# AHzZ123/orb_slam2_with_comment

Hardware: AMD Instinct MI355X
Metric: frames/sec (Track+LocalMap) on 1241×376 stereo; kpts+desc/sec at 1/2/4/8 GPUs (higher is better)
Workload: dtype u8; 1 GPU; Track+LocalMap per stereo frame: ORBextractor(L,R) [2000 feat, 1.2, 8 lv, FAST 20/7] + ComputeStereoMatches + TrackWithMotionModel [SearchByProjection(CF,LF,th=7), PoseOptimization] + TrackLocalMap [SearchLocalPoints(th=1, ~1971 MPs), PoseOptimization] + LocalMapping::Run every 4th frame on the concurrent LocalMapping thread [ProcessNewKeyFrame: KeyFrame::ComputeBoW (a queued keyframe's issued bes; frames_resident=8, parallelism=one stereo stream per GPU x1

## Files before the change

orb_slam2_with_comment_amd/csrc/lba.hip:

```cpp
#include <algorithm>
#include <cfloat>
#include <chrono>
#include <cstdio>
#include <cstdlib>
#include <cmath>
#include <cstring>
#include <new>
#include <thread>
#include <vector>

#include "extractor.h"
#include "se3_device.h"
#include "wave_ops.h"

#if defined(__HIP_DEVICE_COMPILE__) && !defined(__gfx950__)
#error "lba.hip's fence-free fan-ins are validated on gfx950 only"
#endif

#pragma clang fp contract(fast)

namespace orbmi {

constexpr int kBaMaxPoses = 30;
constexpr int kBaMaxN = 6 * kBaMaxPoses;
// ... 172 lines not shown
    edge_robust_math(fl, ed, edge_chi2_math(ed, err), &r0, &r1);
    *w = (fl & 2) ? info : r1 * info;
    const double s = (fl & 2) ? 1.0 : r1;
    for (int k = 0; k < 3; k++) om[k] = -(info * err[k]) * s;
}

__device__ inline void edge_error_at(const BaDev& a, int i, const double* T, const double* Xp, double* err) {
    const orbmi_ba_edge e = a.edges[i];
    edge_err_math(e, ba_cam(a.kfs[e.kf]), T + 8 * e.kf, Xp, err);
}

__device__ inline void edge_error(const BaDev& a, int i, const double* T, const double* X, double* err) {
    edge_error_at(a, i, T, X + 4 * a.edges[i].point, err);
}

__device__ inline double edge_chi2(const BaDev& a, int i) { return edge_chi2_math(a.edges[i], a.err + 3 * i); }

__device__ inline void edge_robust(const BaDev& a, int i, double c, double* rho0, double* rho1) {
    edge_robust_math(a.eflag[i], a.edges[i], c, rho0, rho1);
}

template <int NT>
__device__ inline double block_sum(double v, double* red) {
    for (int o = 32; o > 0; o >>= 1) v += __shfl_xor(v, o, 64);
    if ((threadIdx.x & 63) == 0) red[threadIdx.x >> 6] = v;
    __syncthreads();
    double t = 0;
    for (int w = 0; w < NT / 64; w++) t += red[w];
    __syncthreads();
    return t;
}

template <int NT>
__device__ inline void block_sum2_t0(double& x, double& y, double* red ) {
    for (int o = 32; o > 0; o >>= 1) {
        x += __shfl_xor(x, o, 64);
        y += __shfl_xor(y, o, 64);
    }
    if ((threadIdx.x & 63) == 0) {
        red[threadIdx.x >> 6] = x;
        red[NT / 64 + (threadIdx.x >> 6)] = y;
    }
    __syncthreads();
    if (threadIdx.x == 0) {
        x = 0;
        y = 0;
        for (int w = 0; w < NT / 64; w++) x += red[w];
        for (int w = 0; w < NT / 64; w++) y += red[NT / 64 + w];
    }
}

template <int NT>
__device__ inline double block_max(double v, double* red) {
    for (int o = 32; o > 0; o >>= 1) v = fmax(v, __shfl_xor(v, o, 64));
    if ((threadIdx.x & 63) == 0) red[threadIdx.x >> 6] = v;
    __syncthreads();
    double t = 0;
    for (int w = 0; w < NT / 64; w++) t = fmax(t, red[w]);
    __syncthreads();
    return t;
}

__device__ inline int packed(int r, int c, int N) { return r * N - r * (r - 1) / 2 + (c - r); }

__host__ __device__ inline int mfma_tile_pos(int T, int R, int C) {
    const int i = R >> 4, j = C >> 4, rr = R & 15;
    return (i * (T + 1) - i * (i - 1) / 2 + (j - i)) * 256 + (rr >> 2) * 64 + 16 * (rr & 3) + (C & 15);
}


__device__ inline bool point_active(const BaDev& a, int p) {
    for (int i = a.pt_start[p]; i < a.pt_start[p + 1]; i++)
        if (a.eflag[i] & 4) return true;
    return false;
}

__device__ inline bool ba_check_stop(const BaDev& a, BaCtl& c) {
    const int idx = c.checks++;
    const bool s = (a.stop && *a.stop) || (a.stop_at >= 0 && idx >= a.stop_at);
    if (s && c.stop_seen < 0) c.stop_seen = idx;
    return s;
}

__global__ __launch_bounds__(kBaBlock) void k_ba_setup(BaDev a, double* __restrict__ T, double* __restrict__ X,
                                                       unsigned char* __restrict__ out_erase) {
    const int i = blockIdx.x * blockDim.x + threadIdx.x;
    if (i == 0) {
        BaCtl c = {};
        c.checks = 1;
        c.stop_seen = -1;
        *a.ctl = c;
        for (int k = 0; k < 8; k++) a.istat[k] = 0;
    }
    if (i < a.nkf) {
        const float* t = a.kfs[i].tcw;
        double R[3][3];
        for (int r = 0; r < 3; r++)
            for (int c = 0; c < 3; c++) R[r][c] = t[4 * r + c];
        Q q = q_from_matrix(R);
        q_normalize(q);
        double* Ti = T + 8 * i;
        Ti[0] = q.x; Ti[1] = q.y; Ti[2] = q.z; Ti[3] = q.w; Ti[4] = t[3]; Ti[5] = t[7]; Ti[6] = t[11]; Ti[7] = 0;
        a.kf_act[i] = 0;
    }
    if (i < a.nf) a.arrive_kf[i] = 0;
    if (i < a.npt) {
        for (int r = 0; r < 3; r++) X[4 * i + r] = a.pts[i].pos[r];
        X[4 * i + 3] = 0;
    }
    if (i < a.nedge) {
        a.eflag[i] = 0;
        out_erase[i] = 0;
        a.err[3 * i] = a.err[3 * i + 1] = a.err[3 * i + 2] = 0;
    }
}

__global__ __launch_bounds__(kBaBlock) void k_ba_levels(BaDev a) {
    if (!(a.ctl->phases_done >= 1 && a.ctl->do_more)) return;
    const int i = blockIdx.x * blockDim.x + threadIdx.x;
    const double* T = a.Tb[a.ctl->cur];
    const double* X = a.Xb[a.ctl->cur];
    if (i >= a.nedge) return;
    const orbmi_ba_edge e = a.edges[i];
    if (a.pts[e.point].bad) return;
    double p[3];
    se3_map(T + 8 * e.kf, X + 4 * e.point, p);
    const double th = edge_stereo(e) ? 7.815 : 5.991;
    unsigned char f = a.eflag[i] & 3;
    if (edge_chi2(a, i) > th || !(p[2] > 0.0)) f |= 1;
    f |= 2;
    a.eflag[i] = f;
}

__device__ inline void activate_ctl_body(const BaDev& a, int max_it, int gen);
__global__ __launch_bounds__(kBaBlock) void k_ba_activate_edges(BaDev a, int max_it, int gen) {
    if (gen > 1 && !(a.ctl->phases_done >= gen - 1 && a.ctl->do_more)) return;
    __shared__ double red[kBaBlock / 64];
    const int i = blockIdx.x * blockDim.x + threadIdx.x;
    int first = 0;
    if (i < a.nedge) {
        unsigned char f = a.eflag[i] & 3;
        if (!(f & 1)) {
            f |= 4;
            const orbmi_ba_edge e = a.edges[i];
            a.kf_act[e.kf] = gen;
            first = 1;
            for (int j = a.pt_start[e.point]; j < i; j++)
                if (!(a.eflag[j] & 1)) { first = 0; break; }
        }
        a.eflag[i] = f;
    }
    const double n = block_sum<kBaBlock>((double)first, red);
    __shared__ bool last;
    if (threadIdx.x == 0) {
        a.part_lin[blockIdx.x] = n;
        __threadfence();
        last = atomicAdd(&a.ctl->arrive_e, 1u) == gridDim.x - 1;
    }
    __syncthreads();
    if (!last) return;
    __threadfence();
    if (threadIdx.x < 64) activate_ctl_body(a, max_it, gen);
    if (threadIdx.x == 0) a.ctl->arrive_e = 0;
}

__device__ inline void activate_ctl_body(const BaDev& a, int max_it, int gen) {
    const int lane = threadIdx.x;
    double c = 0;
    for (int b = lane; b < a.nb_e; b += 64) c += a.part_lin[b];
    const int nl = (int)wave_sum(c);
    int n = 0;
    for (int o0 = 0; o0 < a.nkf; o0 += 64) {
        const int oi = o0 + lane;
        int k = -1;
        bool take = false;
        if (oi < a.nkf) {
            k = a.kf_order[oi];
            take = !a.kfs[k].fixed && a.kf_act[k] == gen;
        }
        const unsigned long long m = __ballot(take);
        const int idx = n + __popcll(m & ((1ull << lane) - 1));
        if (k >= 0) {
            a.pose_idx[k] = take && idx < kBaMaxPoses ? idx : -1;
            if (take && idx < kBaMaxPoses) a.pose_kf[idx] = k;
        }
        n += __popcll(m);
    }
    if (lane == 0) {
        a.istat[0] = n;
        a.istat[1] = nl;
        a.istat[2] = n > kBaMaxPoses;
        BaCtl& c2 = *a.ctl;
        c2.np = min(n, kBaMaxPoses);
        c2.nl = nl;
        c2.unsupported |= n > kBaMaxPoses;
// ... 1310 lines not shown
        for (int e = pe0 + j; e < pe1; e += kBaUpdLanes) {
            act += (a.eflag[e] & 4) ? 1.0 : 0.0;
            const int i1 = a.e_pi[e];
            if (i1 < 0) continue;
            const double* B = y.Hpl + 18 * (long long)e;
            const double* xp = a.xp + 6 * i1;
#pragma unroll
            for (int r = 0; r < 6; r++) {
                c0 += B[r * 3] * xp[r];
                c1 += B[r * 3 + 1] * xp[r];
                c2 += B[r * 3 + 2] * xp[r];
            }
        }
        c0 = sum8(c0); c1 = sum8(c1); c2 = sum8(c2); act = sum8(act);
        if (own && j == 0) {
            double xl[3] = {0, 0, 0};
            if (ok && act > 0) {
                const double cl[3] = {y.bl[3 * p] - c0, y.bl[3 * p + 1] - c1, y.bl[3 * p + 2] - c2};
                double Di[9];
                point_dinv(y.Hll, p, lam, Di);
                for (int r = 0; r < 3; r++) xl[r] = Di[r * 3] * cl[0] + Di[r * 3 + 1] * cl[1] + Di[r * 3 + 2] * cl[2];
            }
            for (int r = 0; r < 3; r++) {
                const double x = X[4 * p + r] + xl[r];
                Xt[4 * p + r] = x;
                xs[ps][r] = x;
                if (ok) sc += xl[r] * (lam * xl[r] + y.bl[3 * p + r]);
            }
        }
    }
    __syncthreads();
    const bool lds = be1 - be0 <= kBaUpdLdsEdges;
    for (int e = e_pre; e < be1; e += blockDim.x) {
        EdgeIn s;
        if (e == e_pre) s = pre;
        else edge_in(a, e, Tt, s);
        chi += edge_trial(a, t, e, s, &xs[s.e.point - p0][0], lds ? sHe + 9 * (e - be0) : nullptr);
    }
    __syncthreads();
    {
        double h[9] = {0, 0, 0, 0, 0, 0, 0, 0, 0};
        for (int e = pe0 + j; e < pe1; e += kBaUpdLanes) {
            if (!(a.eflag[e] & 4)) continue;
            const double* He = lds ? sHe + 9 * (e - be0) : t.Hle + 9 * (long long)e;
#pragma unroll
            for (int k = 0; k < 9; k++) h[k] += He[k];
        }
#pragma unroll
        for (int k = 0; k < 9; k++) h[k] = sum8(h[k]);
        if (own && j == 0) {
            double* H = t.Hll + 9 * p;
            H[0] = h[0]; H[1] = h[1]; H[2] = h[2];
            H[3] = h[1]; H[4] = h[3]; H[5] = h[4];
            H[6] = h[2]; H[7] = h[4]; H[8] = h[5];
            for (int k = 0; k < 3; k++) t.bl[3 * p + k] = h[6 + k];
        }
    }
    block_sum2_t0<kBaUpdThreads>(chi, sc, red);
    if (tid == 0) {
        __hip_atomic_store(&part_chi[blockIdx.x], chi, __ATOMIC_RELAXED, __HIP_MEMORY_SCOPE_AGENT);
        __hip_atomic_store(&part_scale[blockIdx.x], sc, __ATOMIC_RELAXED, __HIP_MEMORY_SCOPE_AGENT);
        asm volatile("s_waitcnt vmcnt(0)" ::: "memory");
        last = atomicAdd(&ctl.arrive, 1u) == gridDim.x - 1;
    }
    __syncthreads();
    if (!last) return;
    if (tid < 64) k_ba_control_body(a);
    if (tid == 0) ctl.arrive = 0;
}

__device__ inline void chi_body(const BaDev& a, int phase) {
    const double chi = wave_sum_fixed_sc1(a.part_lin, a.nb_e);
    if (threadIdx.x == 0) {
        BaCtl& c = *a.ctl;
        c.chi_out[phase] = chi;
        c.it_out[phase] = (c.np + c.nl == 0) ? -1 : c.it;
        c.phases_done = phase + 1;
        if (phase == 0) c.do_more = !ba_check_stop(a, c);
    }
}

__global__ __launch_bounds__(kBaBlock) void k_ba_finish(BaDev a, float* __restrict__ out_tcw,
                                                        float* __restrict__ out_pos,
                                                        unsigned char* __restrict__ out_erase) {
    const int i = blockIdx.x * blockDim.x + threadIdx.x;
    const double* T = a.Tb[a.ctl->cur];
    const double* X = a.Xb[a.ctl->cur];
    if (i < a.nedge) {
        const orbmi_ba_edge e = a.edges[i];
        if (!a.pts[e.point].bad) {
            double p[3];
            se3_map(T + 8 * e.kf, X + 4 * e.point, p);
            const double th = edge_stereo(e) ? 7.815 : 5.991;
            out_erase[i] = (edge_chi2(a, i) > th || !(p[2] > 0.0)) ? 1 : 0;
        }
    }
    if (i < a.nkf) {
        const double* Ti = T + 8 * i;
        double R[3][3];
        q_to_matrix(load_q(Ti), R);
        float* o = out_tcw + 16 * i;
        for (int r = 0; r < 3; r++) {
            for (int c = 0; c < 3; c++) o[4 * r + c] = (float)R[r][c];
            o[4 * r + 3] = (float)Ti[4 + r];
        }
        o[12] = 0; o[13] = 0; o[14] = 0; o[15] = 1;
    }
    if (i < a.npt)
        for (int r = 0; r < 3; r++) out_pos[3 * i + r] = (float)X[4 * i + r];
}

}

struct orbmi_ba {
    int device = 0;
    hipStream_t stream = nullptr;
    bool own_stream = true;
    hipEvent_t done = nullptr;
    uint8_t* d_buf = nullptr;
    size_t cap = 0;
    uint8_t* h_stage = nullptr;
    size_t cap_stage = 0;
    hipEvent_t up_done = nullptr;
    hipStream_t up_stream = nullptr;
    uint8_t* h_out = nullptr;
    size_t cap_out = 0;
    orbmi::BaCtl* h_ctl = nullptr;
    int* h_stop = nullptr;
    int* d_stop = nullptr;
    int stop_at = -1;
    void (*enqueued)(void*) = nullptr;
    void* enqueued_arg = nullptr;
};

namespace {

using namespace orbmi;

struct BaTrace {
    bool on = getenv("ORBMI_BA_TRACE") != nullptr;
    std::chrono::steady_clock::time_point t0 = std::chrono::steady_clock::now(), last = t0;
    char buf[512];
    int n = 0;
    void mark(const char* what) {
        if (!on) return;
        const auto t = std::chrono::steady_clock::now();
        n += snprintf(buf + n, sizeof(buf) - n > 0 ? sizeof(buf) - n : 0, " %s %.1f", what,
                      std::chrono::duration<double, std::micro>(t - last).count());
        last = t;
    }
    ~BaTrace() {
        if (on) fprintf(stderr, "[ba] total %.1f us:%s\n",
                        std::chrono::duration<double, std::micro>(std::chrono::steady_clock::now() - t0).count(), buf);
    }
};

inline bool stop_set(const volatile int* stop) { return stop && __atomic_load_n(stop, __ATOMIC_ACQUIRE) != 0; }

bool ba_block_table(int nf, std::vector<int>& blk_id) {
    const int nblk = nf * (nf + 1) / 2;
    blk_id.assign(std::max(nblk, 1), -1);
    const int R = 8;
    std::vector<int> load(R, 0), grp(std::max(nf, 1));
    for (int r = 0; r < nf; r++) {
        const int g = (int)(std::min_element(load.begin(), load.end()) - load.begin());
        grp[r] = g;
        load[g] += nf - r;
    }
    std::vector<int> next(R);
    for (int g = 0; g < R; g++) next[g] = g;
    std::vector<char> used(std::max(nblk, 1), 0);
    std::vector<int> spill;
    int l = 0;
    for (int ra = 0; ra < nf; ra++)
        for (int rb = ra; rb < nf; rb++, l++) {
            const int g = grp[ra];
            if (next[g] < nblk) { blk_id[l] = next[g]; used[next[g]] = 1; next[g] += R; }
            else spill.push_back(l);
        }
    int free_id = 0;
    for (int x : spill) {
        while (free_id < nblk && used[free_id]) free_id++;
        if (free_id >= nblk) return false;
        blk_id[x] = free_id;
        used[free_id] = 1;
    }
    std::vector<char> hit(std::max(nblk, 1), 0);
    for (int x = 0; x < nblk; x++) {
        const int id = blk_id[x];
        if (id < 0 || id >= nblk || hit[id]) return false;
        hit[id] = 1;
    }
    return true;
}

constexpr int kBaStepSlack = 1;

struct Runner {
    orbmi_ba& h;
    BaDev a;
    const volatile int* stop;

    void launch_solve() {
        static_assert((6 * kBaSolveMfmaMaxPoses + 15) / 16 <= 8, "a case per tile count below");
        switch (a.mfma_T) {
#define ORBMI_MFMA_CASE(T_) \
    case T_: hipLaunchKernelGGL(k_ba_solve_mfma<T_>, dim3(1), dim3(kBaMfmaThreads), 0, h.stream, a); break;
            ORBMI_MFMA_CASE(1) ORBMI_MFMA_CASE(2) ORBMI_MFMA_CASE(3) ORBMI_MFMA_CASE(4)
            ORBMI_MFMA_CASE(5) ORBMI_MFMA_CASE(6) ORBMI_MFMA_CASE(7) ORBMI_MFMA_CASE(8)
#undef ORBMI_MFMA_CASE
            default: hipLaunchKernelGGL(k_ba_solve, dim3(1), dim3(kBaSolveThreads), 0, h.stream, a); break;
        }
    }

    int wait() {
        ORBMI_HIP(hipEventRecord(h.done, h.stream));
        if (!stop) {
            ORBMI_HIP(hipEventSynchronize(h.done));
            return ORBMI_OK;
        }
        for (;;) {
            *(volatile int*)h.h_stop = stop_set(stop) ? 1 : 0;
            const hipError_t e = hipEventQuery(h.done);
            if (e == hipSuccess) return ORBMI_OK;
            if (e != hipErrorNotReady) return ORBMI_E_HIP;
            std::this_thread::yield();
        }
    }

    int read_ctl() {
        ORBMI_HIP(hipMemcpyAsync(h.h_ctl, a.ctl, sizeof(BaCtl), hipMemcpyDeviceToHost, h.stream));
        return wait();
    }

    void step(int gen) {
        a.run_gen = gen;
        if (a.nblk > 0)
            hipLaunchKernelGGL(k_ba_schur, dim3(a.nblk + kSchurKfSplit * a.nf + (a.mfma_T > 0)), dim3(kSchurThreads), 0,
                               h.stream, a);
        launch_solve();
        hipLaunchKernelGGL(k_ba_update_errors, dim3(a.nb_q), dim3(kBaUpdThreads), 0, h.stream, a);
    }

    void prologue(int iterations, int gen) {
        a.run_gen = gen;
        if (gen == 2) hipLaunchKernelGGL(k_ba_levels, dim3(a.nb_e), dim3(kBaBlock), 0, h.stream, a);
        hipLaunchKernelGGL(k_ba_activate_edges, dim3(a.nb_e), dim3(kBaBlock), 0, h.stream, a, iterations, gen);
        hipLaunchKernelGGL(k_ba_linearize, dim3(a.nb_e), dim3(kBaBlock), 0, h.stream, a);
        hipLaunchKernelGGL(k_ba_reduce, dim3(a.nb_p + std::max(a.nf, 1)), dim3(kBaBlock), 0, h.stream, a);
    }

    void epilogue(int gen) {
        a.run_gen = gen;
        hipLaunchKernelGGL(k_ba_errors, dim3(a.nb_e), dim3(kBaBlock), 0, h.stream, a, gen - 1);
    }
};

}

extern "C" {

int orbmi_ba_create(int device, orbmi_ba** out) {
    if (!out) return ORBMI_E_ARG;
    *out = nullptr;
    int ndev = 0;
    if (hipGetDeviceCount(&ndev) != hipSuccess || device < 0 || device >= ndev) return ORBMI_E_HIP;
    orbmi_ba* b = new (std::nothrow) orbmi_ba();
    if (!b) return ORBMI_E_ARG;
    b->device = device;
    if (hipSetDevice(device) != hipSuccess || orbmi::stream_create(&b->stream, "BA") != hipSuccess ||
        hipEventCreateWithFlags(&b->done, hipEventDisableTiming) != hipSuccess ||
        hipEventCreateWithFlags(&b->up_done, hipEventDisableTiming) != hipSuccess ||
        hipHostMalloc((void**)&b->h_ctl, sizeof(BaCtl)) != hipSuccess ||
        hipHostMalloc((void**)&b->h_stop, 64, hipHostMallocMapped | hipHostMallocCoherent) != hipSuccess ||
        hipHostGetDevicePointer((void**)&b->d_stop, b->h_stop, 0) != hipSuccess) {
        orbmi_ba_destroy(b);
        return ORBMI_E_HIP;
    }
    *b->h_stop = 0;
    *out = b;
    return ORBMI_OK;
}

void orbmi_ba_destroy(orbmi_ba* b) {
    if (!b) return;
    (void)hipSetDevice(b->device);
    if (b->stream) (void)hipStreamSynchronize(b->stream);
    if (b->d_buf) (void)hipFree(b->d_buf);
    if (b->h_stage) (void)hipHostFree(b->h_stage);
    if (b->h_ctl) (void)hipHostFree(b->h_ctl);
    if (b->h_stop) (void)hipHostFree(b->h_stop);
    if (b->done) (void)hipEventDestroy(b->done);
    if (b->up_stream) {
        (void)hipStreamSynchronize(b->up_stream);
        (void)hipStreamDestroy(b->up_stream);
    }
    if (b->up_done) (void)hipEventDestroy(b->up_done);
    if (b->h_out) (void)hipHostFree(b->h_out);
    if (b->stream && b->own_stream) (void)hipStreamDestroy(b->stream);
    delete b;
}

int orbmi_debug_ba_schur_blocks(int nf, int* table, int cap, int* n_out) {
    if (nf < 0 || nf > kBaMaxPoses || !n_out) return ORBMI_E_ARG;
    const int nblk = nf * (nf + 1) / 2, nb = nblk + kSchurKfSplit * nf + 1;
    *n_out = nb;
    if (cap < nb || !table) return ORBMI_E_CAP;
    std::vector<int> blk_id;
    if (!ba_block_table(nf, blk_id)) return ORBMI_E_UNSUPPORTED;
    std::vector<int> ra_of(std::max(nblk, 1)), rb_of(std::max(nblk, 1)), l_of(std::max(nblk, 1));
    for (int ra = 0, l = 0; ra < nf; ra++)
        for (int rb = ra; rb < nf; rb++, l++) { ra_of[blk_id[l]] = ra; rb_of[blk_id[l]] = rb; l_of[blk_id[l]] = l; }
    for (int b = 0; b < nb; b++) {
        const SchurRole role = schur_role(b, nblk, nf);
        int* t = table + 4 * b;
        t[0] = role.kind;
        t[1] = role.kind == 0 ? ra_of[role.r] : role.kind == 1 ? role.r : -1;
        t[2] = role.kind == 0 ? rb_of[role.r] : role.kind == 1 ? role.h : -1;
        t[3] = role.kind == 0 ? l_of[role.r] : -1;
    }
    return ORBMI_OK;
}

int orbmi_ba_set_stop_at_check(orbmi_ba* b, int k) {
    if (!b) return ORBMI_E_ARG;
    b->stop_at = k < 0 ? -1 : k;
    return ORBMI_OK;
}

int orbmi_ba_set_enqueued_hook(orbmi_ba* b, void (*fn)(void*), void* arg) {
    if (!b) return ORBMI_E_ARG;
    b->enqueued = fn;
    b->enqueued_arg = arg;
    return ORBMI_OK;
}

int orbmi_ba_set_stream(orbmi_ba* b, void* stream) {
    if (!b) return ORBMI_E_ARG;
    ORBMI_HIP(hipSetDevice(b->device));
    ORBMI_HIP(hipStreamSynchronize(b->stream));
    hipStream_t s = (hipStream_t)stream;
    if (!s) ORBMI_HIP(orbmi::stream_create(&s, "BA"));
    if (b->own_stream) ORBMI_HIP(hipStreamDestroy(b->stream));
    b->stream = s;
    b->own_stream = stream == nullptr;
    return ORBMI_OK;
}

int orbmi_local_bundle_adjustment(orbmi_ba* b, const orbmi_ba_problem* P, orbmi_ba_result* R,
                                  const volatile int* stop) {
    if (!b || !P || !R || P->nkf < 0 || P->npt < 0 || P->nedge < 0) return ORBMI_E_ARG;
    if ((P->nkf && (!P->kfs || !R->tcw)) || (P->npt && (!P->pts || !R->pos)) || (P->nedge && (!P->edges || !R->erase)))
        return ORBMI_E_ARG;
    orbmi_ba& h = *b;
    BaTrace tr;
    ORBMI_HIP(hipSetDevice(h.device));
    R->aborted = 0;
    R->iterations[0] = R->iterations[1] = 0;
    R->chi2[0] = R->chi2[1] = 0;
    R->stop_check = -1;
    R->checks = 1;
    for (int i = 0; i < P->nedge; i++) R->erase[i] = 0;
    if (stop_set(stop) || h.stop_at == 0) {
        R->aborted = 1;
        R->stop_check = 0;
        return ORBMI_OK;
    }
    const int nkf = P->nkf, npt = P->npt, ne = P->nedge;
    if (nkf > kBaMaxKf) return ORBMI_E_UNSUPPORTED;
    {
        std::vector<int> last_pt(std::max(nkf, 1), -1);
        for (int i = 0; i < ne; i++) {
            const orbmi_ba_edge& e = P->edges[i];
// ... 5 lines not shown
    }
    std::vector<int> order(std::max(nkf, 1));
    for (int k = 0; k < nkf; k++) order[k] = k;
    std::stable_sort(order.begin(), order.begin() + nkf, [&](int x, int y) { return P->kfs[x].id < P->kfs[y].id; });
    std::vector<int> rank(std::max(nkf, 1), -1), free_kf;
    for (int oi = 0; oi < nkf; oi++)
        if (!P->kfs[order[oi]].fixed) { rank[order[oi]] = (int)free_kf.size(); free_kf.push_back(order[oi]); }
    const int nf = (int)free_kf.size();
    const long long nblk_ll = (long long)nf * (nf + 1) / 2;
    if (nblk_ll > (1 << 20)) return ORBMI_E_UNSUPPORTED;
    const int nblk = (int)nblk_ll;
    std::vector<int> blk_id;
    if (!ba_block_table(nf, blk_id)) return ORBMI_E_UNSUPPORTED;
    auto blk_of = [nf, &blk_id](int ra, int rb) { return blk_id[ra * nf - ra * (ra - 1) / 2 + (rb - ra)]; };
    const int nb_e = std::max(1, (ne + kBaBlock - 1) / kBaBlock), nb_p = std::max(1, (npt + kBaBlock - 1) / kBaBlock);
    const int nb_q = std::max(1, (npt + kBaUpdPts - 1) / kBaUpdPts);
    auto al = [](size_t x) { return (x + 255) & ~(size_t)255; };
    size_t off = 0;
    auto take = [&](size_t bytes) { size_t o = off; off += al(std::max(bytes, (size_t)8)); return o; };
    const size_t o_kfs = take(sizeof(orbmi_ba_keyframe) * nkf), o_pts = take(sizeof(orbmi_ba_point) * npt),
                 o_edges = take(sizeof(orbmi_ba_edge) * ne), o_order = take(4 * nkf), o_pts_start = take(4 * (npt + 1)),
                 o_kfs_start = take(4 * (nkf + 1)), o_kf_edges = take(4 * (size_t)ne), o_kf_pos = take(4 * (size_t)ne),
                 o_kf_pt = take(4 * (size_t)ne), o_blk_kf = take(8 * (size_t)nblk), o_free = take(4 * (size_t)nf);
    const size_t up_bytes = off;
    hipStream_t s = h.stream;
    ORBMI_HIP(hipEventSynchronize(h.up_done));
    if (up_bytes > h.cap_stage) {
        if (h.h_stage) (void)hipHostFree(h.h_stage);
        h.h_stage = nullptr;
        h.cap_stage = 0;
        ORBMI_HIP(hipHostMalloc((void**)&h.h_stage, up_bytes));
        h.cap_stage = up_bytes;
    }
    uint8_t* S = h.h_stage;
    int* pt_start = (int*)(S + o_pts_start);
    int* kf_start = (int*)(S + o_kfs_start);
    int* kf_edges = (int*)(S + o_kf_edges);
    int* kf_pos = (int*)(S + o_kf_pos);
    int* kf_pt = (int*)(S + o_kf_pt);
    std::memset(pt_start, 0, 4 * (size_t)(npt + 1));
    std::memset(kf_start, 0, 4 * (size_t)(nkf + 1));
    for (int i = 0; i < ne; i++) { pt_start[P->edges[i].point + 1]++; kf_start[P->edges[i].kf + 1]++; }
    for (int p = 0; p < npt; p++) pt_start[p + 1] += pt_start[p];
    for (int k = 0; k < nkf; k++) kf_start[k + 1] += kf_start[k];
    long long npair_cap = 0;
    {
        std::vector<int> fill(kf_start, kf_start + nkf);
        int p = -1;
        long long m = 0;
        for (int i = 0; i < ne; i++) {
            const orbmi_ba_edge& e = P->edges[i];
            const int j = fill[e.kf]++;
            kf_pos[i] = j;
            kf_edges[j] = i;
            kf_pt[j] = e.point;
            if (e.point != p) { npair_cap += m * m; m = 0; p = e.point; }
            m += rank[e.kf] >= 0;
        }
        npair_cap += m * m;
    }
    if (npair_cap > (1LL << 28)) return ORBMI_E_UNSUPPORTED;
    const int npair = (int)npair_cap;
    if (nkf) std::memcpy(S + o_order, order.data(), 4 * (size_t)nkf);
    if (nf) std::memcpy(S + o_free, free_kf.data(), 4 * (size_t)nf);
    {
        int* bk = (int*)(S + o_blk_kf);
        for (int ra = 0; ra < nf; ra++)
            for (int rb = ra; rb < nf; rb++) { bk[2 * blk_of(ra, rb)] = free_kf[ra]; bk[2 * blk_of(ra, rb) + 1] = free_kf[rb]; }
    }
    auto put = [&](size_t o, const void* src, size_t bytes) { if (bytes) std::memcpy(S + o, src, bytes); };
    put(o_kfs, P->kfs, sizeof(orbmi_ba_keyframe) * nkf);
    put(o_pts, P->pts, sizeof(orbmi_ba_point) * npt);
    put(o_edges, P->edges, sizeof(orbmi_ba_edge) * ne);
    const size_t o_blk_cnt = take(4 * (size_t)nblk), o_blk_start = take(4 * ((size_t)nblk + 1)),
                 o_pairs = take(8 * (size_t)npair), o_pairpt = take(4 * (size_t)npair);
    const size_t o_e_pi = take(4 * (size_t)ne), o_T0 = take(64 * nkf), o_T1 = take(64 * nkf), o_X0 = take(32 * npt),
                 o_X1 = take(32 * npt), o_err = take(24 * (size_t)ne), o_eflag = take(ne), o_pidx = take(4 * nkf), o_kfact = take(4 * nkf),
                 o_pkf = take(4 * kBaMaxPoses), o_Hpl = take(2 * 144 * (size_t)ne), o_Hle = take(2 * 72 * (size_t)ne),
                 o_Hpe = take(2 * 216 * (size_t)ne), o_Hll = take(2 * 72 * npt), o_bl = take(2 * 24 * npt),
                 o_Hpp = take(288 * kBaMaxPoses), o_bp = take(48 * kBaMaxPoses), o_S = take(8 * (size_t)kBaPacked),
                 o_bs = take(8 * kBaMaxN), o_xp = take(8 * kBaMaxN), o_scal = take(64), o_plin = take(8 * (size_t)nb_e),
                 o_ptchi = take(8 * (size_t)nb_q), o_ptsc = take(8 * (size_t)nb_q),
                 o_pmax = take(8 * ((size_t)nb_p + kBaMaxPoses)), o_istat = take(32), o_ctl = take(sizeof(BaCtl)),
                 o_otcw = take(64 * nkf), o_opos = take(12 * npt), o_oerase = take(ne),
                 o_pkfs = take(8 * 64 * kSchurKfSplit * (size_t)kBaMaxPoses), o_arrkf = take(4 * kBaMaxPoses);
    if (off > h.cap) {
        if (h.d_buf) (void)hipFree(h.d_buf);
        h.d_buf = nullptr;
        h.cap = 0;
        ORBMI_HIP(hipMalloc((void**)&h.d_buf, off));
        h.cap = off;
    }
    uint8_t* B = h.d_buf;
    tr.mark("host_index");
    if (!h.up_stream) ORBMI_HIP(orbmi::stream_create(&h.up_stream, "BA"));
    ORBMI_HIP(hipMemcpyAsync(B, S, up_bytes, hipMemcpyHostToDevice, h.up_stream));
    ORBMI_HIP(hipEventRecord(h.up_done, h.up_stream));
    ORBMI_HIP(hipStreamWaitEvent(s, h.up_done, 0));
    const size_t out_bytes = o_oerase + (size_t)std::max(ne, 1) - o_otcw;
    if (out_bytes > h.cap_out) {
        if (h.h_out) (void)hipHostFree(h.h_out);
        h.h_out = nullptr;
        h.cap_out = 0;
        ORBMI_HIP(hipHostMalloc((void**)&h.h_out, out_bytes));
        h.cap_out = out_bytes;
    }
    uint8_t* const Ho = h.h_out;
    BaDev a;
    a.nkf = nkf; a.npt = npt; a.nedge = ne; a.nblk = nblk; a.nf = nf;
    a.nb_e = nb_e; a.nb_p = nb_p; a.nb_q = nb_q;
    a.ctl = (BaCtl*)(B + o_ctl);
    a.stop = stop ? h.d_stop : nullptr;
    a.stop_at = h.stop_at;
    *(volatile int*)h.h_stop = stop_set(stop) ? 1 : 0;
    a.Tb[0] = (double*)(B + o_T0); a.Tb[1] = (double*)(B + o_T1);
    a.Xb[0] = (double*)(B + o_X0); a.Xb[1] = (double*)(B + o_X1);
    a.part_lin = (double*)(B + o_plin); a.part_tchi = (double*)(B + o_ptchi); a.part_tscale = (double*)(B + o_ptsc);
    a.part_max = (double*)(B + o_pmax);
    a.kfs = (const orbmi_ba_keyframe*)(B + o_kfs);
    a.pts = (const orbmi_ba_point*)(B + o_pts);
    a.edges = (const orbmi_ba_edge*)(B + o_edges);
    a.kf_order = (const int*)(B + o_order);
    a.free_kf = (const int*)(B + o_free);
    a.part_kf = (double*)(B + o_pkfs);
    a.arrive_kf = (unsigned*)(B + o_arrkf);
    a.pt_start = (const int*)(B + o_pts_start);
    a.kf_start = (const int*)(B + o_kfs_start);
    a.kf_edges = (const int*)(B + o_kf_edges);
    a.kf_pos = (const int*)(B + o_kf_pos);
    a.kf_pt = (const int*)(B + o_kf_pt);
    a.e_pi = (int*)(B + o_e_pi);
    a.blk_kf = (const int*)(B + o_blk_kf);
    a.blk_cnt = (int*)(B + o_blk_cnt);
    a.blk_start = (int*)(B + o_blk_start);
    a.blk_pairs = (int2*)(B + o_pairs);
    a.blk_pt = (int*)(B + o_pairpt);
    a.err = (double*)(B + o_err); a.eflag = B + o_eflag;
    a.pose_idx = (int*)(B + o_pidx); a.pose_kf = (int*)(B + o_pkf); a.kf_act = (int*)(B + o_kfact);
    for (int L = 0; L < 2; L++) {
        a.Hplb[L] = (double*)(B + o_Hpl) + (size_t)L * 18 * ne;
        a.Hleb[L] = (double*)(B + o_Hle) + (size_t)L * 9 * ne;
        a.Hpeb[L] = (double*)(B + o_Hpe) + (size_t)L * 27 * ne;
        a.Hllb[L] = (double*)(B + o_Hll) + (size_t)L * 9 * npt;
        a.blb[L] = (double*)(B + o_bl) + (size_t)L * 3 * npt;
    }
    a.Hpl = a.Hplb[0]; a.Hle = a.Hleb[0]; a.Hpe = a.Hpeb[0]; a.Hll = a.Hllb[0]; a.bl = a.blb[0];
    a.Hpp = (double*)(B + o_Hpp); a.bp = (double*)(B + o_bp);
    a.S = (double*)(B + o_S); a.bs = (double*)(B + o_bs); a.xp = (double*)(B + o_xp);
    a.scal = (double*)(B + o_scal); a.istat = (int*)(B + o_istat);
    a.mfma_T = nf <= kBaSolveMfmaMaxPoses ? std::max(1, (6 * nf + 15) / 16) : 0;
    Runner r{h, a, stop};
    unsigned char* out_erase = B + o_oerase;
    const int nb_all = std::max(1, (std::max(std::max(nkf, npt), ne) + kBaBlock - 1) / kBaBlock);
    hipLaunchKernelGGL(k_ba_setup, dim3(nb_all), dim3(kBaBlock), 0, s, a, a.Tb[0], a.Xb[0], out_erase);
    if (nblk > 0) {
        hipLaunchKernelGGL(k_ba_pairs_count, dim3(nblk), dim3(kPairThreads), 0, s, a);
        hipLaunchKernelGGL(k_ba_pairs_fill, dim3(nblk), dim3(kPairThreads), 0, s, a);
    }
    ORBMI_HIP(hipGetLastError());
    tr.mark("enqueue_setup");
    const char* slack_env = getenv("ORBMI_BA_SLACK");
    const int slack = slack_env ? std::max(0, atoi(slack_env)) : kBaStepSlack;
    auto enqueue = [&](int from, int more) {
        if (from == 0) r.prologue(5, 1);
        if (from <= 1) {
            for (int k = 0; k < (from == 0 ? 5 + slack : more); k++) r.step(1);
            r.epilogue(1);
            r.prologue(10, 2);
        }
        for (int k = 0; k < (from <= 1 ? 10 + slack : more); k++) r.step(2);
        r.epilogue(2);
        hipLaunchKernelGGL(k_ba_finish, dim3(nb_all), dim3(kBaBlock), 0, s, a, (float*)(B + o_otcw), (float*)(B + o_opos),
                           out_erase);
        hipError_t e = hipSuccess;
        if (e == hipSuccess) e = hipMemcpyAsync(Ho, B + o_otcw, o_oerase + ne - o_otcw, hipMemcpyDeviceToHost, s);
        return e;
    };
    int rc, from = 0, more = 0;
    for (;;) {
        ORBMI_HIP(enqueue(from, more));
        ORBMI_HIP(hipGetLastError());
        if (from == 0 && h.enqueued) h.enqueued(h.enqueued_arg);
        if ((rc = r.read_ctl())) return rc;
        const BaCtl& c = *h.h_ctl;
        if (c.unsupported) return ORBMI_E_UNSUPPORTED;
        if (c.phases_done >= 2 || (c.phases_done == 1 && !c.do_more)) break;
        from = c.phases_done == 0 ? 1 : 2;
        more = std::max(1, c.max_it - c.it);
        tr.mark(from == 1 ? "resume5" : "resume10");
    }
    tr.mark("optimize+finish");
    if (nkf) std::memcpy(R->tcw, Ho, 64 * (size_t)nkf);
    if (npt) std::memcpy(R->pos, Ho + (o_opos - o_otcw), 12 * (size_t)npt);
    if (ne) std::memcpy(R->erase, Ho + (o_oerase - o_otcw), (size_t)ne);
    const BaCtl& c = *h.h_ctl;
    const bool second = c.do_more != 0;
    R->iterations[0] = c.it_out[0];
    R->iterations[1] = second ? c.it_out[1] : 0;
    R->chi2[0] = c.chi_out[0];
    R->chi2[1] = second ? c.chi_out[1] : 0;
    R->stop_check = c.stop_seen;
    R->checks = c.checks;
    return ORBMI_OK;
}

}
```

orb_slam2_with_comment_amd/csrc/matcher.hip:

```cpp
#include <algorithm>

#include <cstring>

#include "matcher.h"
#include "track_update.h"
#include "tri_geom.h"
#include "wave_ops.h"

namespace orbmi {

constexpr int kGridCols = 64, kGridRows = 48, kGridCells = kGridCols * kGridRows;
constexpr int TH_HIGH = 100, TH_LOW = 50, HISTO_LENGTH = 30;


__device__ inline int popc_desc(const uint8_t* a, const uint8_t* b) {
    const uint4* x = reinterpret_cast<const uint4*>(a);
    const uint4* y = reinterpret_cast<const uint4*>(b);
    return popc256(x[0], x[1], y[0], y[1]);
}

__device__ inline void grid_build_block(const DevFrame& F, int* __restrict__ cell_start, int* __restrict__ cell_list,
                                        int* __restrict__ kp_cell) {
    __shared__ int cnt[kGridCells + 1];
    __shared__ int scratch[20];
    const int tid = threadIdx.x;
    for (int i = tid; i < kGridCells; i += blockDim.x) cnt[i] = 0;
    __syncthreads();
    const int n = frame_n(F);
    for (int i = tid; i < n; i += blockDim.x) {
        const orbmi_keypoint kp = F.keys[i];
        const int px = (int)roundf((kp.x - F.min_x) * F.grid_w_inv);
        const int py = (int)roundf((kp.y - F.min_y) * F.grid_h_inv);
        int c = -1;
        if (!(px < 0 || px >= kGridCols || py < 0 || py >= kGridRows)) { c = px * kGridRows + py; atomicAdd(&cnt[c], 1); }
        kp_cell[i] = c;
    }
    __syncthreads();
    int v[3], s = 0;
    for (int k = 0; k < 3; k++) { v[k] = cnt[tid * 3 + k]; s += v[k]; }
    int total;
    int e = block_excl_scan(s, scratch, &total);
    for (int k = 0; k < 3; k++) { cell_start[tid * 3 + k] = e; cnt[tid * 3 + k] = e; e += v[k]; }
    if (tid == 0) cell_start[kGridCells] = total;
    __syncthreads();
    for (int i = tid; i < n; i += blockDim.x) {
        const int c = kp_cell[i];
        if (c >= 0) cell_list[atomicAdd(&cnt[c], 1)] = i;
    }
}

__global__ __launch_bounds__(1024) void k_grid_build(DevFrame F, int* __restrict__ cell_start,
                                                     int* __restrict__ cell_list, int* __restrict__ kp_cell,
                                                     const int* gate, int gate_min) {
    if (gate && *gate >= gate_min) return;
    grid_build_block(F, cell_start, cell_list, kp_cell);
}

__global__ __launch_bounds__(1024) void k_grid_build_multi(const FuseKF* __restrict__ kfs, int* __restrict__ kp_cell,
                                                           int ncap) {
    const FuseKF& K = kfs[blockIdx.x];
    if (threadIdx.x == 0) *K.ncand = 0;
    grid_build_block(K.F, const_cast<int*>(K.cs), const_cast<int*>(K.cl), kp_cell + (size_t)blockIdx.x * ncap);
}

template <int G = 1, class Fn>
__device__ inline void for_features_in_area(const DevFrame& F, const int* cell_start, const int* cell_list,
                                            float x, float y, float r, int minLevel, int maxLevel, int glane, Fn fn) {
    const int nMinCellX = max(0, (int)floorf((x - F.min_x - r) * F.grid_w_inv));
    if (nMinCellX >= kGridCols) return;
    const int nMaxCellX = min(kGridCols - 1, (int)ceilf((x - F.min_x + r) * F.grid_w_inv));
    if (nMaxCellX < 0) return;
    const int nMinCellY = max(0, (int)floorf((y - F.min_y - r) * F.grid_h_inv));
    if (nMinCellY >= kGridRows) return;
    const int nMaxCellY = min(kGridRows - 1, (int)ceilf((y - F.min_y + r) * F.grid_h_inv));
    if (nMaxCellY < 0) return;
    const bool bCheckLevels = (minLevel > 0) || (maxLevel >= 0);
    const int ny = nMaxCellY - nMinCellY + 1, ncell = (nMaxCellX - nMinCellX + 1) * ny;
    for (int ci = glane; ci < ncell; ci += G) {
        const int c = (nMinCellX + ci / ny) * kGridRows + nMinCellY + ci % ny;
        for (int j = cell_start[c]; j < cell_start[c + 1]; j++) {
            const int idx = cell_list[j];
            const orbmi_keypoint kp = F.keys[idx];
            if (bCheckLevels) {
                if (kp.octave < minLevel) continue;
                if (maxLevel >= 0 && kp.octave > maxLevel) continue;
            }
            const float distx = kp.x - x, disty = kp.y - y;
            if (fabsf(distx) < r && fabsf(disty) < r) fn(idx, c);
        }
    }
}
template <class Fn>
__device__ inline void for_features_in_area(const DevFrame& F, const int* cell_start, const int* cell_list,
                                            float x, float y, float r, int minLevel, int maxLevel, Fn fn) {
    for_features_in_area<1>(F, cell_start, cell_list, x, y, r, minLevel, maxLevel, 0, fn);
}

__device__ inline unsigned long long cand_entry(int dist, int cell, int idx) {
    return ((unsigned long long)dist << 40) | ((unsigned long long)cell << 20) | (unsigned)idx;
}

__device__ inline void transform(const float* T, const float* p, float* o) {
#pragma unroll
    for (int r = 0; r < 3; r++) o[r] = ((T[4 * r] * p[0] + T[4 * r + 1] * p[1]) + T[4 * r + 2] * p[2]) + T[4 * r + 3];
}
__device__ inline void camera_center(const float* T, float* o) {
#pragma unroll
    for (int c = 0; c < 3; c++) o[c] = -((T[c] * T[3] + T[4 + c] * T[7]) + T[8 + c] * T[11]);
}

__device__ inline orbmi_mappoint_track frustum_record(const DevFrame& F, const Pose34& T, const orbmi_mappoint& mp,
                                                      float viewingCosLimit) {
    orbmi_mappoint_track t = {0, 0.f, 0.f, 0.f, 0, 0.f};
    bool ok = !(mp.flags & (ORBMI_MP_BAD | ORBMI_MP_SEEN));
    float Pc[3], Ow[3], u = 0, v = 0, invz = 0, dist = 0, viewCos = 0;
    if (ok) {
        transform(T.m, mp.pos, Pc);
        ok = !(Pc[2] < 0.0f);
    }
    if (ok) {
        invz = 1.0f / Pc[2];
        u = F.fx * Pc[0] * invz + F.cx;
        v = F.fy * Pc[1] * invz + F.cy;
        ok = !(u < F.min_x || u > F.max_x) && !(v < F.min_y || v > F.max_y);
    }
    if (ok) {
        camera_center(T.m, Ow);
        const float maxDistance = 1.2f * mp.max_distance, minDistance = 0.8f * mp.min_distance;
        const float PO[3] = {mp.pos[0] - Ow[0], mp.pos[1] - Ow[1], mp.pos[2] - Ow[2]};
        dist = (float)sqrt((double)PO[0] * PO[0] + (double)PO[1] * PO[1] + (double)PO[2] * PO[2]);
        ok = !(dist < minDistance || dist > maxDistance);
        if (ok) {
            const double dot = (double)PO[0] * mp.normal[0] + (double)PO[1] * mp.normal[1] + (double)PO[2] * mp.normal[2];
            viewCos = (float)(dot / (double)dist);
            ok = !(viewCos < viewingCosLimit);
        }
    }
    if (ok) {
        const float ratio = mp.max_distance / dist;
        int nScale = (int)ceilf((float)log((double)ratio) / F.log_scale_factor);
        if (nScale < 0) nScale = 0;
        else if (nScale >= F.nlevels) nScale = F.nlevels - 1;
        t.in_view = 1;
        t.proj_x = u;
        t.proj_xr = u - F.bf * invz;
        t.proj_y = v;
        t.level = nScale;
        t.view_cos = viewCos;
    }
    return t;
}

__global__ __launch_bounds__(256) void k_frustum(DevFrame F, const orbmi_mappoint* __restrict__ mps, int n,
                                                 float viewingCosLimit, orbmi_mappoint_track* __restrict__ tr,
                                                 int* __restrict__ n_in_view) {
    const int i = blockIdx.x * blockDim.x + threadIdx.x;
    if (i >= n) return;
    const orbmi_mappoint mp = mps[i];
    const Pose34 T = frame_pose(F);
    const orbmi_mappoint_track t = frustum_record(F, T, mp, viewingCosLimit);
// ... 96 lines not shown
    int* n_in_view;
    const orbmi_lastframe_point* lfp;
    float th;
    int mono;
    unsigned long long* cand;
    int* ncand;
    unsigned long long* top;
    const int* gate;
    int gate_min;
};

struct Window {
    float x, y, r, ur;
    int minL, maxL;
    const uint8_t* desc;
};

__device__ inline bool local_window(const CandArgs& a, const orbmi_mappoint& mp, const orbmi_mappoint_track& t,
                                    Window* w) {
    int level;
    if (!local_query(a.F, mp, t, a.th, &w->x, &w->y, &w->r, &level)) return false;
    w->minL = level - 1;
    w->maxL = level;
    w->ur = t.proj_xr;
    w->desc = mp.desc;
    return true;
}

__device__ inline bool make_window(const CandArgs& a, int q, const float* Tc, bool fw, bool bw, Window* w) {
    if (a.mode == 0) return local_window(a, a.mps[q], a.tr[q], w);
    const orbmi_lastframe_point& p = a.lfp[q];
    LfQuery lq;
    if (!lf_query(a.F, Tc, a.LF, p, q, a.th, fw, bw, &lq)) return false;
    w->x = lq.u; w->y = lq.v; w->r = lq.radius; w->ur = lq.ur; w->minL = lq.minL; w->maxL = lq.maxL;
    w->desc = p.desc;
    return true;
}

template <int G, bool FR = false>
__global__ __launch_bounds__(256) void k_candidates(CandArgs a) {
    constexpr int NG = 256 / G, cap = Matcher::kCandCap;
    __shared__ unsigned long long buf[NG][cap];
    __shared__ int cnt[NG];
    const int gl = threadIdx.x / G, lane = threadIdx.x % G;
    const int q = blockIdx.x * NG + gl;
    if (a.gate && *a.gate >= a.gate_min) return;
    const int nq = a.mode == 1 ? frame_n(a.LF) : a.nq;
    Pose34 Tc;
    bool fw = false, bw = false;
    if (a.mode == 1) {
        Tc = frame_pose(a.F);
        motion_direction(a.F, Tc.m, a.LF, a.mono, &fw, &bw);
    }
    Window w;
    bool valid = false;
    if constexpr (FR) {
        if (q < nq) {
            const orbmi_mappoint& mp = a.mps[q];
            const Pose34 T = frame_pose(a.F);
            const orbmi_mappoint_track t = frustum_record(a.F, T, mp, a.frustum_cos);
            if (lane == 0) {
                a.tr_out[q] = t;
                if (t.in_view && a.n_in_view) atomicAdd(a.n_in_view, 1);
            }
            valid = local_window(a, mp, t, &w);
        }
    } else {
        valid = q < nq && make_window(a, q, Tc.m, fw, bw, &w);
    }
    if (lane == 0) cnt[gl] = 0;
    __builtin_amdgcn_fence(__ATOMIC_RELEASE, "wavefront");
    __builtin_amdgcn_wave_barrier();
    if (valid) {
        const DevFrame& F = a.F;
        const int nMinCellX = max(0, (int)floorf((w.x - F.min_x - w.r) * F.grid_w_inv));
        const int nMaxCellX = min(kGridCols - 1, (int)ceilf((w.x - F.min_x + w.r) * F.grid_w_inv));
        const int nMinCellY = max(0, (int)floorf((w.y - F.min_y - w.r) * F.grid_h_inv));
        const int nMaxCellY = min(kGridRows - 1, (int)ceilf((w.y - F.min_y + w.r) * F.grid_h_inv));
        if (nMinCellX < kGridCols && nMaxCellX >= 0 && nMinCellY < kGridRows && nMaxCellY >= 0) {
            const int ny = nMaxCellY - nMinCellY + 1, ncell = (nMaxCellX - nMinCellX + 1) * ny;
            const bool bCheckLevels = (w.minL > 0) || (w.maxL >= 0);
            const uint4* md = reinterpret_cast<const uint4*>(w.desc);
            const uint4 m0 = md[0], m1 = md[1];
            for (int ci = lane; ci < ncell; ci += G) {
                const int c = (nMinCellX + ci / ny) * kGridRows + nMinCellY + ci % ny;
                for (int j = a.cs[c]; j < a.cs[c + 1]; j++) {
                    const int idx = a.cl[j];
                    const orbmi_keypoint kp = F.keys[idx];
                    if (bCheckLevels) {
                        if (kp.octave < w.minL) continue;
                        if (w.maxL >= 0 && kp.octave > w.maxL) continue;
                    }
                    if (!(fabsf(kp.x - w.x) < w.r && fabsf(kp.y - w.y) < w.r)) continue;
                    if (F.u_right && F.u_right[idx] > 0 && fabsf(w.ur - F.u_right[idx]) > w.r) continue;
                    const uint4* fd = reinterpret_cast<const uint4*>(F.desc + 32 * (long long)idx);
                    const int pos = atomicAdd(&cnt[gl], 1);
                    if (pos < cap) buf[gl][pos] = cand_entry(popc256(m0, m1, fd[0], fd[1]), c, idx);
                }
            }
        }
    }
    __builtin_amdgcn_fence(__ATOMIC_RELEASE, "wavefront");
    __builtin_amdgcn_wave_barrier();
    __builtin_amdgcn_fence(__ATOMIC_ACQUIRE, "wavefront");
    const int n = cnt[gl], nk = min(n, cap);
    unsigned long long last = 0;
    for (int k = 0; k < kTopK; k++) {
        unsigned long long m = ~0ull;
        for (int p = lane; p < nk; p += G) {
            const unsigned long long e = buf[gl][p];
            if ((k == 0 || e > last) && e < m) m = e;
        }
        if constexpr (G == 16) {
            unsigned long long v;
            v = dpp_mov_u64<kDppXor1>(m); m = v < m ? v : m;
            v = dpp_mov_u64<kDppXor2>(m); m = v < m ? v : m;
            v = dpp_mov_u64<kDppHalfMirror>(m); m = v < m ? v : m;
            v = dpp_mov_u64<kDppRor8>(m); m = v < m ? v : m;
        } else {
#pragma unroll
            for (int o = G / 2; o > 0; o >>= 1) {
                const unsigned long long v = __shfl_xor(m, o, G);
                m = v < m ? v : m;
            }
        }
        if (valid && lane == 0) a.top[(long long)q * kTopK + k] = m;
        last = m;
    }
    if (valid && n > kTopK)
        for (int p = lane; p < nk; p += G) a.cand[(long long)q * cap + p] = buf[gl][p];
    if (q < nq && lane == 0) a.ncand[q] = valid ? n : 0;
}

struct GreedyArgs {
    int mode;
    int nq;
    const unsigned long long* cand;
    const int* ncand;
    const unsigned long long* top;
    int cap;
    const uint8_t* occ0;
    DevFrame F;
    DevFrame LF;
    const int* cs;
    const int* cl;
    const orbmi_mappoint* mps;
    const orbmi_mappoint_track* tr;
    const orbmi_lastframe_point* lfp;
    float th, nnratio;
    int mono, check_ori;
    int* res;
    int* out;
    int* nmatches;
    const int* gate;
    int gate_min;
};

constexpr int kGreedyMaxKp = 16384;
constexpr int kGreedyRounds = 48;

template <class Occ>
__device__ inline int greedy_eval(const GreedyArgs& a, int q, const float* Tc, bool fw, bool bw, Occ occ) {
    unsigned long long b1 = ~0ull, b2 = ~0ull;
    auto take = [&](unsigned long long e) {
        if (occ((int)(e & 0xFFFFF))) return;
        if (e < b1) { b2 = b1; b1 = e; }
        else if (e < b2) b2 = e;
    };
    const int nc = a.ncand[q];
    const unsigned long long* t = a.top + (long long)q * kTopK;
    const int kk = nc <= a.cap ? min(nc, kTopK) : 0;
    for (int k = 0; k < kk && b2 == ~0ull; k++) take(t[k]);
    if (b2 == ~0ull && nc > kTopK) {
        b1 = b2 = ~0ull;
        if (nc <= a.cap) {
            const unsigned long long* c = a.cand + (long long)q * a.cap;
            for (int k0 = 0; k0 < nc; k0 += 16) {
                unsigned long long e[16];
#pragma unroll
                for (int j = 0; j < 16; j++) e[j] = k0 + j < nc ? c[k0 + j] : ~0ull;
#pragma unroll
                for (int j = 0; j < 16; j++)
// ... 1583 lines not shown
```

Before: 3129 frames/s.

## Write BA outputs to mapped host memory and balance matcher cell loops across lanes

The bundle adjustment finish kernel now writes poses, points, erase flags and the control block straight into coherent mapped host memory, so the trailing device-to-host memcpy and the separate control readback go away. In the matcher, the per-lane loop over grid cells is replaced by a group-wide prefix-sum scheduler. It spreads candidate features evenly across the 8 or 16 lanes and processes two items per lane per step, with prefetched cell ranges and loads issued ahead of use. A schur launch guard is also widened. These trade PCIe copy latency for zero-copy writes, and per-lane load imbalance for shared-memory staging and wave barriers.

```diff
diff --git a/orb_slam2_with_comment_amd/csrc/lba.hip b/orb_slam2_with_comment_amd/csrc/lba.hip
--- a/orb_slam2_with_comment_amd/csrc/lba.hip
+++ b/orb_slam2_with_comment_amd/csrc/lba.hip
@@ -278,8 +278,7 @@
     return s;
 }
 
-__global__ __launch_bounds__(kBaBlock) void k_ba_setup(BaDev a, double* __restrict__ T, double* __restrict__ X,
-                                                       unsigned char* __restrict__ out_erase) {
+__global__ __launch_bounds__(kBaBlock) void k_ba_setup(BaDev a, double* __restrict__ T, double* __restrict__ X) {
     const int i = blockIdx.x * blockDim.x + threadIdx.x;
     if (i == 0) {
         BaCtl c = {};
@@ -306,7 +305,6 @@
     }
     if (i < a.nedge) {
         a.eflag[i] = 0;
-        out_erase[i] = 0;
         a.err[3 * i] = a.err[3 * i + 1] = a.err[3 * i + 2] = 0;
     }
 }
@@ -1783,18 +1781,22 @@
 
 __global__ __launch_bounds__(kBaBlock) void k_ba_finish(BaDev a, float* __restrict__ out_tcw,
                                                         float* __restrict__ out_pos,
-                                                        unsigned char* __restrict__ out_erase) {
+                                                        unsigned char* __restrict__ out_erase,
+                                                        BaCtl* __restrict__ out_ctl) {
     const int i = blockIdx.x * blockDim.x + threadIdx.x;
     const double* T = a.Tb[a.ctl->cur];
     const double* X = a.Xb[a.ctl->cur];
+    if (i == 0) *out_ctl = *a.ctl;
     if (i < a.nedge) {
         const orbmi_ba_edge e = a.edges[i];
+        unsigned char erase = 0;
         if (!a.pts[e.point].bad) {
             double p[3];
             se3_map(T + 8 * e.kf, X + 4 * e.point, p);
             const double th = edge_stereo(e) ? 7.815 : 5.991;
-            out_erase[i] = (edge_chi2(a, i) > th || !(p[2] > 0.0)) ? 1 : 0;
-        }
+            erase = (edge_chi2(a, i) > th || !(p[2] > 0.0)) ? 1 : 0;
+        }
+        out_erase[i] = erase;
     }
     if (i < a.nkf) {
         const double* Ti = T + 8 * i;
@@ -1825,6 +1827,7 @@
     hipEvent_t up_done = nullptr;
     hipStream_t up_stream = nullptr;
     uint8_t* h_out = nullptr;
+    uint8_t* d_out = nullptr;
     size_t cap_out = 0;
     orbmi::BaCtl* h_ctl = nullptr;
     int* h_stop = nullptr;
@@ -1929,14 +1932,11 @@
         }
     }
 
-    int read_ctl() {
-        ORBMI_HIP(hipMemcpyAsync(h.h_ctl, a.ctl, sizeof(BaCtl), hipMemcpyDeviceToHost, h.stream));
-        return wait();
-    }
+    int read_ctl() { return wait(); }
 
     void step(int gen) {
         a.run_gen = gen;
-        if (a.nblk > 0)
+        if (a.nblk > 0 || a.mfma_T > 0)
             hipLaunchKernelGGL(k_ba_schur, dim3(a.nblk + kSchurKfSplit * a.nf + (a.mfma_T > 0)), dim3(kSchurThreads), 0,
                                h.stream, a);
         launch_solve();
@@ -1972,7 +1972,6 @@
     if (hipSetDevice(device) != hipSuccess || orbmi::stream_create(&b->stream, "BA") != hipSuccess ||
         hipEventCreateWithFlags(&b->done, hipEventDisableTiming) != hipSuccess ||
         hipEventCreateWithFlags(&b->up_done, hipEventDisableTiming) != hipSuccess ||
-        hipHostMalloc((void**)&b->h_ctl, sizeof(BaCtl)) != hipSuccess ||
         hipHostMalloc((void**)&b->h_stop, 64, hipHostMallocMapped | hipHostMallocCoherent) != hipSuccess ||
         hipHostGetDevicePointer((void**)&b->d_stop, b->h_stop, 0) != hipSuccess) {
         orbmi_ba_destroy(b);
@@ -1989,7 +1988,6 @@
     if (b->stream) (void)hipStreamSynchronize(b->stream);
     if (b->d_buf) (void)hipFree(b->d_buf);
     if (b->h_stage) (void)hipHostFree(b->h_stage);
-    if (b->h_ctl) (void)hipHostFree(b->h_ctl);
     if (b->h_stop) (void)hipHostFree(b->h_stop);
     if (b->done) (void)hipEventDestroy(b->done);
     if (b->up_stream) {
@@ -2161,7 +2159,6 @@
                  o_bs = take(8 * kBaMaxN), o_xp = take(8 * kBaMaxN), o_scal = take(64), o_plin = take(8 * (size_t)nb_e),
                  o_ptchi = take(8 * (size_t)nb_q), o_ptsc = take(8 * (size_t)nb_q),
                  o_pmax = take(8 * ((size_t)nb_p + kBaMaxPoses)), o_istat = take(32), o_ctl = take(sizeof(BaCtl)),
-                 o_otcw = take(64 * nkf), o_opos = take(12 * npt), o_oerase = take(ne),
                  o_pkfs = take(8 * 64 * kSchurKfSplit * (size_t)kBaMaxPoses), o_arrkf = take(4 * kBaMaxPoses);
     if (off > h.cap) {
         if (h.d_buf) (void)hipFree(h.d_buf);
@@ -2176,15 +2173,19 @@
     ORBMI_HIP(hipMemcpyAsync(B, S, up_bytes, hipMemcpyHostToDevice, h.up_stream));
     ORBMI_HIP(hipEventRecord(h.up_done, h.up_stream));
     ORBMI_HIP(hipStreamWaitEvent(s, h.up_done, 0));
-    const size_t out_bytes = o_oerase + (size_t)std::max(ne, 1) - o_otcw;
+    const size_t ho_pos = al(64 * (size_t)std::max(nkf, 1)), ho_erase = ho_pos + al(12 * (size_t)std::max(npt, 1)),
+                 ho_ctl = ho_erase + al((size_t)std::max(ne, 1)), out_bytes = ho_ctl + sizeof(BaCtl);
     if (out_bytes > h.cap_out) {
         if (h.h_out) (void)hipHostFree(h.h_out);
-        h.h_out = nullptr;
+        h.h_out = h.d_out = nullptr;
         h.cap_out = 0;
-        ORBMI_HIP(hipHostMalloc((void**)&h.h_out, out_bytes));
+        ORBMI_HIP(hipHostMalloc((void**)&h.h_out, out_bytes, hipHostMallocMapped | hipHostMallocCoherent));
+        ORBMI_HIP(hipHostGetDevicePointer((void**)&h.d_out, h.h_out, 0));
         h.cap_out = out_bytes;
     }
     uint8_t* const Ho = h.h_out;
+    uint8_t* const Do = h.d_out;
+    h.h_ctl = (BaCtl*)(Ho + ho_ctl);
     BaDev a;
     a.nkf = nkf; a.npt = npt; a.nedge = ne; a.nblk = nblk; a.nf = nf;
     a.nb_e = nb_e; a.nb_p = nb_p; a.nb_q = nb_q;
@@ -2229,9 +2230,8 @@
     a.scal = (double*)(B + o_scal); a.istat = (int*)(B + o_istat);
     a.mfma_T = nf <= kBaSolveMfmaMaxPoses ? std::max(1, (6 * nf + 15) / 16) : 0;
     Runner r{h, a, stop};
-    unsigned char* out_erase = B + o_oerase;
     const int nb_all = std::max(1, (std::max(std::max(nkf, npt), ne) + kBaBlock - 1) / kBaBlock);
-    hipLaunchKernelGGL(k_ba_setup, dim3(nb_all), dim3(kBaBlock), 0, s, a, a.Tb[0], a.Xb[0], out_erase);
+    hipLaunchKernelGGL(k_ba_setup, dim3(nb_all), dim3(kBaBlock), 0, s, a, a.Tb[0], a.Xb[0]);
     if (nblk > 0) {
         hipLaunchKernelGGL(k_ba_pairs_count, dim3(nblk), dim3(kPairThreads), 0, s, a);
         hipLaunchKernelGGL(k_ba_pairs_fill, dim3(nblk), dim3(kPairThreads), 0, s, a);
@@ -2249,11 +2249,9 @@
         }
         for (int k = 0; k < (from <= 1 ? 10 + slack : more); k++) r.step(2);
         r.epilogue(2);
-        hipLaunchKernelGGL(k_ba_finish, dim3(nb_all), dim3(kBaBlock), 0, s, a, (float*)(B + o_otcw), (float*)(B + o_opos),
-                           out_erase);
-        hipError_t e = hipSuccess;
-        if (e == hipSuccess) e = hipMemcpyAsync(Ho, B + o_otcw, o_oerase + ne - o_otcw, hipMemcpyDeviceToHost, s);
-        return e;
+        hipLaunchKernelGGL(k_ba_finish, dim3(nb_all), dim3(kBaBlock), 0, s, a, (float*)Do, (float*)(Do + ho_pos),
+                           Do + ho_erase, (BaCtl*)(Do + ho_ctl));
+        return hipSuccess;
     };
     int rc, from = 0, more = 0;
     for (;;) {
@@ -2270,8 +2268,8 @@
     }
     tr.mark("optimize+finish");
     if (nkf) std::memcpy(R->tcw, Ho, 64 * (size_t)nkf);
-    if (npt) std::memcpy(R->pos, Ho + (o_opos - o_otcw), 12 * (size_t)npt);
-    if (ne) std::memcpy(R->erase, Ho + (o_oerase - o_otcw), (size_t)ne);
+    if (npt) std::memcpy(R->pos, Ho + ho_pos, 12 * (size_t)npt);
+    if (ne) std::memcpy(R->erase, Ho + ho_erase, (size_t)ne);
     const BaCtl& c = *h.h_ctl;
     const bool second = c.do_more != 0;
     R->iterations[0] = c.it_out[0];
diff --git a/orb_slam2_with_comment_amd/csrc/matcher.hip b/orb_slam2_with_comment_amd/csrc/matcher.hip
--- a/orb_slam2_with_comment_amd/csrc/matcher.hip
+++ b/orb_slam2_with_comment_amd/csrc/matcher.hip
@@ -63,6 +63,61 @@
     grid_build_block(K.F, const_cast<int*>(K.cs), const_cast<int*>(K.cl), kp_cell + (size_t)blockIdx.x * ncap);
 }
 
+template <int G, class Load, class Use>
+__device__ inline void for_window_items(const int* __restrict__ cell_start, const int* __restrict__ cell_list,
+                                        int nMinCellX, int nMinCellY, int ny, int ncell, int glane, Load load, Use use) {
+    static_assert(G == 8 || G == 16, "a group is 8 or 16 lanes");
+    __shared__ int s_cnt[256];
+    __shared__ int2 s_sc[256];
+    const int tid = threadIdx.x, gb = tid - glane;
+    auto cell_range = [&](int ci, int* n, int2* sc) {
+        *n = 0;
+        *sc = make_int2(0, 0);
+        if (ci < ncell) {
+            const int c = (nMinCellX + ci / ny) * kGridRows + nMinCellY + ci % ny;
+            const int s = cell_start[c], e = cell_start[c + 1];
+            *n = e - s;
+            *sc = make_int2(s, c);
+        }
+    };
+    int n;
+    int2 sc;
+    cell_range(glane, &n, &sc);
+    for (int c0 = 0; c0 < ncell; c0 += G) {
+        int n_next;
+        int2 sc_next;
+        cell_range(c0 + G + glane, &n_next, &sc_next);
+        s_cnt[tid] = n;
+        s_sc[tid] = sc;
+        __builtin_amdgcn_fence(__ATOMIC_RELEASE, "wavefront");
+        __builtin_amdgcn_wave_barrier();
+        __builtin_amdgcn_fence(__ATOMIC_ACQUIRE, "wavefront");
+        int incl[G], total = 0;
+#pragma unroll
+        for (int l = 0; l < G; l++) { total += s_cnt[gb + l]; incl[l] = total; }
+        for (int t = glane; t < total; t += 2 * G) {
+            const bool two = t + G < total;
+            const int t2 = two ? t + G : t;
+            int o = 0, o2 = 0, ex = 0, ex2 = 0;
+#pragma unroll
+            for (int l = 0; l < G; l++) {
+                if (incl[l] <= t) { o++; ex = incl[l]; }
+                if (incl[l] <= t2) { o2++; ex2 = incl[l]; }
+            }
+            const int2 a = s_sc[gb + o], b = s_sc[gb + o2];
+            const int idx = cell_list[a.x + (t - ex)], idx2 = cell_list[b.x + (t2 - ex2)];
+            const auto rec = load(idx);
+            const auto rec2 = load(idx2);
+            use(rec, idx, a.y);
+            if (two) use(rec2, idx2, b.y);
+        }
+        __builtin_amdgcn_fence(__ATOMIC_RELEASE, "wavefront");
+        __builtin_amdgcn_wave_barrier();
+        n = n_next;
+        sc = sc_next;
+    }
+}
+
 template <int G = 1, class Fn>
 __device__ inline void for_features_in_area(const DevFrame& F, const int* cell_start, const int* cell_list,
                                             float x, float y, float r, int minLevel, int maxLevel, int glane, Fn fn) {
@@ -76,6 +131,19 @@
     if (nMaxCellY < 0) return;
     const bool bCheckLevels = (minLevel > 0) || (maxLevel >= 0);
     const int ny = nMaxCellY - nMinCellY + 1, ncell = (nMaxCellX - nMinCellX + 1) * ny;
+    if constexpr (G > 1) {
+        for_window_items<G>(
+            cell_start, cell_list, nMinCellX, nMinCellY, ny, ncell, glane, [&](int idx) { return F.keys[idx]; },
+            [&](const orbmi_keypoint& kp, int idx, int c) {
+                if (bCheckLevels) {
+                    if (kp.octave < minLevel) return;
+                    if (maxLevel >= 0 && kp.octave > maxLevel) return;
+                }
+                const float distx = kp.x - x, disty = kp.y - y;
+                if (fabsf(distx) < r && fabsf(disty) < r) fn(idx, c);
+            });
+        return;
+    }
     for (int ci = glane; ci < ncell; ci += G) {
         const int c = (nMinCellX + ci / ny) * kGridRows + nMinCellY + ci % ny;
         for (int j = cell_start[c]; j < cell_start[c + 1]; j++) {
@@ -338,22 +406,28 @@
             const bool bCheckLevels = (w.minL > 0) || (w.maxL >= 0);
             const uint4* md = reinterpret_cast<const uint4*>(w.desc);
             const uint4 m0 = md[0], m1 = md[1];
-            for (int ci = lane; ci < ncell; ci += G) {
-                const int c = (nMinCellX + ci / ny) * kGridRows + nMinCellY + ci % ny;
-                for (int j = a.cs[c]; j < a.cs[c + 1]; j++) {
-                    const int idx = a.cl[j];
-                    const orbmi_keypoint kp = F.keys[idx];
+            struct Item {
+                float x, y, ur;
+                int octave;
+                uint4 d0, d1;
+            };
+            for_window_items<G>(
+                a.cs, a.cl, nMinCellX, nMinCellY, ny, ncell, lane,
+                [&](int idx) {
+                    const orbmi_keypoint& kp = F.keys[idx];
+                    const uint4* fd = reinterpret_cast<const uint4*>(F.desc + 32 * (long long)idx);
+                    return Item{kp.x, kp.y, F.u_right ? F.u_right[idx] : 0.f, kp.octave, fd[0], fd[1]};
+                },
+                [&](const Item& it, int idx, int c) {
                     if (bCheckLevels) {
-                        if (kp.octave < w.minL) continue;
-                        if (w.maxL >= 0 && kp.octave > w.maxL) continue;
+                        if (it.octave < w.minL) return;
+                        if (w.maxL >= 0 && it.octave > w.maxL) return;
                     }
-                    if (!(fabsf(kp.x - w.x) < w.r && fabsf(kp.y - w.y) < w.r)) continue;
-                    if (F.u_right && F.u_right[idx] > 0 && fabsf(w.ur - F.u_right[idx]) > w.r) continue;
-                    const uint4* fd = reinterpret_cast<const uint4*>(F.desc + 32 * (long long)idx);
+                    if (!(fabsf(it.x - w.x) < w.r && fabsf(it.y - w.y) < w.r)) return;
+                    if (F.u_right && it.ur > 0 && fabsf(w.ur - it.ur) > w.r) return;
                     const int pos = atomicAdd(&cnt[gl], 1);
-                    if (pos < cap) buf[gl][pos] = cand_entry(popc256(m0, m1, fd[0], fd[1]), c, idx);
-                }
-            }
+                    if (pos < cap) buf[gl][pos] = cand_entry(popc256(m0, m1, it.d0, it.d1), c, idx);
+                });
         }
     }
     __builtin_amdgcn_fence(__ATOMIC_RELEASE, "wavefront");
```

After: 3205 frames/s (median of 6 runs). 1.02x the previous value.
